# SJTU-ViSYS-team/Avoid-MPC

Hardware: AMD Instinct MI355X
Metric: MPC steps/sec (50k-pt cloud, N=20, 8 obstacle constraints) (higher is better)
Workload: dtype f64; 1 GPU; BASELINE configs[1] batched as configs[2]: 256 scenes/GPU x (50000-pt obstacle cloud + 5000-pt edge cloud, N=20, K=8), fresh frame + zero warm start every step, every in-flight step on its own frames; scenes_per_gpu=256, points=50000, horizon=20, K=8, mpc_max_iter=3, ipm_max_iter=100, streams_in_flight=10, steps_per_launch=4, scenes_per_launch=1024, distinct_frames_bytes=6758400000, hw_queues=4, tie_order=lowest index, parallelism=single GPU, no process group, rccl=no process group (single GPU, plain run): RCCL not used

## Files before the change

avoid_mpc_amd/capi.py:

```python
import ctypes as C
import os

HERE = os.path.dirname(os.path.abspath(__file__))
LIB_PATH = os.path.join(HERE, "libavoid_mpc_amd.so")

AMK_OK, AMK_ERR_INVALID_ARG, AMK_ERR_HIP, AMK_ERR_NO_DEVICE, AMK_ERR_UNSUPPORTED, AMK_ERR_TIMEOUT = 0, 1, 2, 3, 4, 5
AMK_TIES_LOWEST_INDEX, AMK_TIES_NANOFLANN, AMK_TIES_AUTO = 0, 1, 2
AMK_EXACT_OFF, AMK_EXACT_IN_USE, AMK_EXACT_GAVE_UP, AMK_EXACT_TOO_DEEP = -1, 0, 1, 2
AMK_EXACT_NOT_NEEDED = 3
AMK_MAX_K = 64
AMK_MAX_QUERIES = 64
AMK_MAX_HORIZON = 32
AMK_MAX_OUTER_ITER = 8
AMK_MPC_DEFAULT_MAX_ITER = 100

PLUGIN_FUNCTIONS = ["nlp", "nlp_f", "nlp_g", "nlp_grad_f", "nlp_jac_g", "nlp_hess_l", "nlp_grad"]
PLUGIN_HELPERS = ["alloc_mem", "init_mem", "free_mem", "checkout", "release", "incref", "decref", "n_in", "n_out",
                  "default_in", "name_in", "name_out", "sparsity_in", "sparsity_out", "work"]
PLUGIN_SYMBOLS = [f for f in PLUGIN_FUNCTIONS] + [f + "_" + h for f in PLUGIN_FUNCTIONS for h in PLUGIN_HELPERS] + \
                 ["amk_plugin_configure", "amk_plugin_dims"]

SYMBOLS = [
    "amk_version", "amk_status_string", "amk_last_hip_error", "amk_device_count",
    "amk_kd_create", "amk_kd_destroy", "amk_kd_build", "amk_kd_build_pair", "amk_kd_sizes", "amk_kd_search",
# ... 244 lines not shown
        "amk_shard_rccl_info": (i, [C.c_char_p, i, C.POINTER(i), C.POINTER(i)]),
        "amk_shard_wait": (i, [vp, vp, d]),
        "amk_depth_out_size": (i, [i, i, d, C.POINTER(i), C.POINTER(i)]),
        "amk_depth_to_cloud": (i, [vp, i, i, i, C.c_longlong, i, C.POINTER(DepthParams), vp, vp, i, C.c_longlong, vp, vp]),
        "amk_depth_to_cloud_host": (i, [vp, i, i, i, C.c_longlong, i, C.POINTER(DepthParams), vp, vp, i, C.c_longlong, vp]),
        "amk_depth_to_edge_cloud": (i, [vp, i, i, i, C.c_longlong, i, C.POINTER(DepthParams), vp, vp, i, C.c_longlong, vp, vp]),
        "amk_depth_to_edge_cloud_host": (i, [vp, i, i, i, C.c_longlong, i, C.POINTER(DepthParams), vp, vp, i, C.c_longlong, vp]),
        "amk_depth_clouds_work_bytes": (i, [i, i, d, i, C.POINTER(C.c_longlong)]),
        "amk_depth_to_clouds": (i, [vp, i, i, i, C.c_longlong, i, C.POINTER(DepthParams), vp, vp, vp, C.c_longlong, vp, vp, C.c_longlong, vp,
                                    i, vp, C.c_longlong, vp]),
        "amk_depth_to_clouds_host": (i, [vp, i, i, i, C.c_longlong, i, C.POINTER(DepthParams), vp, vp, vp, C.c_longlong, vp, vp, C.c_longlong,
                                         vp, i]),
        "amk_sim_render_depth": (i, [vp, vp, i, i, d, d, C.POINTER(DepthParams), i, i, vp, vp, i, vp]),
        "amk_sim_render_depth_host": (i, [vp, vp, i, i, d, d, C.POINTER(DepthParams), i, i, vp, vp, i]),
        "amk_sim_vehicle_step": (i, [vp, vp, vp, vp, i, d, vp]),
        "amk_sim_vehicle_step_host": (i, [vp, vp, vp, vp, i, d]),
        "amk_sim_render_world": (i, [vp, vp, i, vp, vp, i, i, d, d, C.POINTER(DepthParams), i, i, vp, vp, i, vp]),
        "amk_sim_render_world_host": (i, [vp, vp, i, vp, vp, i, i, d, d, C.POINTER(DepthParams), i, i, vp, vp, i]),
        "amk_sim_vehicle_step_att": (i, [vp, vp, vp, vp, i, d, i, d, vp]),
        "amk_sim_vehicle_step_att_host": (i, [vp, vp, vp, vp, i, d, i, d]),
    }
    sig["amk__kd_set_mode"] = (i, [vp, i])
    sig["amk__sweep_set_target"] = (None, [i])
    sig["amk__sweep_set_order"] = (None, [i])
    sig["amk__frames_force_wide"] = (None, [i])
    sig["amk__mpc_ref_states"] = (i, [vp, vp, ll])
    sig["amk__kfmap_slots_host"] = (i, [vp, vp, vp, vp, vp, vp])
    sig["amk__mpc_dynamics"] = (i, [vp, vp, d, vp, vp, vp, vp])
    sig["amk__depth_set_band_rows"] = (i, [i])
    sig["amk__sim_render_t"] = (i, [vp, vp, i, i, d, d, C.POINTER(DepthParams), i, i, vp, vp, vp])
    sig["amk__sim_chunk"] = (i, [])
    sig["amk__sim_render_world_t"] = (i, [vp, vp, i, vp, vp, i, i, d, d, C.POINTER(DepthParams), i, i, vp, vp, vp])
    sig["amk__sim_world_chunk"] = (i, [])
    for name, (res, args) in sig.items():
        fn = getattr(lib, name, None)
        if fn is None:
            continue
        fn.restype = res
        fn.argtypes = args
    _lib = lib
    return lib


def missing_symbols():
    lib = load()
    return [s for s in SYMBOLS if not hasattr(lib, s)]


def check(status, what=""):
    if status != AMK_OK:
        lib = load()
        msg = lib.amk_status_string(status).decode()
        raise AmkError(f"{what}: {msg} (status {status}, hipError {lib.amk_last_hip_error()})")


def hip_memcpy_dtoh(host_array, dev_ptr):
    import torch
    hip = C.CDLL(os.path.join(os.path.dirname(torch.__file__), "lib", "libamdhip64.so"))
    hip.hipMemcpy.restype = C.c_int
    hip.hipMemcpy.argtypes = [C.c_void_p, C.c_void_p, C.c_size_t, C.c_int]
    return hip.hipMemcpy(host_array.ctypes.data_as(C.c_void_p), C.c_void_p(dev_ptr), host_array.nbytes, 2)


def check_hip(err, what=""):
    if err != 0:
        raise AmkError(f"{what}: hipError {err}")
# ... 30 lines not shown
```

avoid_mpc_amd/csrc/kd_grid.h:

```cpp
#pragma once
#include <cfloat>
#include <type_traits>
#include "kd_device.h"

namespace amk {

#ifndef AMK_GRID_MAX_CELLS
#define AMK_GRID_MAX_CELLS 1024
#endif
constexpr int kGridMaxCells = AMK_GRID_MAX_CELLS;
#ifndef AMK_GRID_PPC
#define AMK_GRID_PPC 64
#endif
constexpr int kGridPointsPerCell = AMK_GRID_PPC;
#ifndef AMK_BUILD_THREADS
#define AMK_BUILD_THREADS 512
#endif
constexpr int kGridBuildThreads = AMK_BUILD_THREADS;
constexpr int kCompactThreads = kGridBuildThreads;
#ifndef AMK_GRID_UNROLL
#define AMK_GRID_UNROLL 16
#endif
constexpr int kGridUnroll = AMK_GRID_UNROLL;
constexpr int kGridParamDoubles = 8;

__device__ __forceinline__ bool finite3(float x, float y, float z) {
    return fabsf(x) <= FLT_MAX && fabsf(y) <= FLT_MAX && fabsf(z) <= FLT_MAX;
}
__device__ __forceinline__ bool boxable3(float x, float y, float z) {
    return fabsf(x) <= 3.0e38f && fabsf(y) <= 3.0e38f && fabsf(z) <= 3.0e38f;
}

__device__ __forceinline__ int cell_of(double p, double bbmin, double inv_h, int g) {
    double c = floor((p - bbmin) * inv_h);
    c = c < 0.0 ? 0.0 : c;
    const double gm = (double)(g - 1);
    c = c > gm ? gm : c;
    return (int)c;
}

__device__ __forceinline__ void grid_geometry(const float *bbox6, int npoints, double *geo, double *gp) {
    double lo[3], hi[3], ext[3], emax = 0.0;
    for (int a = 0; a < 3; ++a) {
        float m0 = bbox6[a], m1 = bbox6[3 + a];
        if (!(m1 >= m0)) { m0 = 0.f; m1 = 0.f; }
        lo[a] = m0; hi[a] = m1;
        ext[a] = (double)m1 - (double)m0;
        emax = fmax(emax, ext[a]);
    }
    const double efloor = fmax(emax * 1e-6, 1e-30);
    double vol = 1.0;
    for (int a = 0; a < 3; ++a) vol *= fmax(ext[a], efloor);
// ... 78 lines not shown
                const int c = hist[i0 + j];
                hist[i0 + j] = run;
                cs[i0 + j] = run;
                run += c;
            }
        if (tid == 0) cs[ncell + 1] = n;
    }
    for (int tt = 1; tt < ntiles; ++tt)
        for (int i = tid; i <= ncell + 1; i += kGridBuildThreads) cs[(size_t)tt * (kGridMaxCells + 2) + i] = n;
    __syncthreads();
    for (int i0 = tid; i0 < n; i0 += kGridUnroll * kGridBuildThreads) {
        float x[kGridUnroll], y[kGridUnroll], z[kGridUnroll];
#pragma unroll
        for (int j = 0; j < kGridUnroll; ++j) {
            const int i = i0 + j * kGridBuildThreads;
            const int ii = i < n ? i : i0;
            x[j] = xs[ii]; y[j] = ys[ii]; z[j] = zs[ii];
        }
#pragma unroll
        for (int j = 0; j < kGridUnroll; ++j) {
            const int i = i0 + j * kGridBuildThreads;
            if (i < n) {
                const int pos = atomicAdd(&hist[cell_id(x[j], y[j], z[j])], 1);
                gpt4[pos] = make_float4(x[j], y[j], z[j], __int_as_float(i));
            }
        }
    }
}

#ifndef AMK_TILE_P
#define AMK_TILE_P 8
#endif
constexpr int kTileP = AMK_TILE_P;
constexpr int kTilePoints = kGridBuildThreads * kTileP;
#ifndef AMK_STAGE_RECORDS
#define AMK_STAGE_RECORDS 4096
#endif
constexpr int kStageRecords = AMK_STAGE_RECORDS;
__host__ __device__ constexpr int grid_tiles(int max_points) { return max_points <= 0 ? 1 : (max_points + kTilePoints - 1) / kTilePoints; }

__device__ __forceinline__ void grid_build_tiles_scene(int s, const float *__restrict__ src, int stride, int cap, int nvis,
                                                       const float *__restrict__ bbox, float4 *__restrict__ GP,
                                                       int *__restrict__ cell_start, int ntiles, double *__restrict__ gparams,
                                                       int *__restrict__ size_out, float *__restrict__ pmax_out,
                                                       float *__restrict__ soa_x = nullptr, float *__restrict__ soa_y = nullptr,
                                                       float *__restrict__ soa_z = nullptr) {
    const int tid = threadIdx.x, lane = tid & 63, w = tid >> 6;
    constexpr int NW = kGridBuildThreads / 64;
    float4 *gpt4 = GP + (size_t)s * cap;
    int *cs_all = cell_start + (size_t)s * ntiles * (kGridMaxCells + 2);
    double *gp = gparams + (size_t)s * kGridParamDoubles;
    __shared__ int hist[kGridMaxCells + 2];
    __shared__ int wsum[NW];
    __shared__ int wcnt[kTileP * NW + 1];
    __shared__ float4 stage[kStageRecords];
    __shared__ float wmax[NW];
    __shared__ double geo[kGridParamDoubles];
    if (tid == 0) grid_geometry(bbox + 6 * s, nvis, geo, gp);
    __syncthreads();
    const double b0 = geo[0], b1 = geo[1], b2 = geo[2], inv_h = geo[4];
    const int g0 = (int)geo[5], g1 = (int)geo[6], g2 = (int)geo[7];
    const int ncell = g0 * g1 * g2;
    float amax = 0.f;
    int kept_before = 0;
    int t = 0;
    for (int i0 = 0; i0 < nvis; i0 += kTilePoints, ++t) {
        int *cs = cs_all + (size_t)t * (kGridMaxCells + 2);
        float x[kTileP], y[kTileP], z[kTileP];
#pragma unroll
        for (int j = 0; j < kTileP; ++j) {
            const int i = i0 + j * kGridBuildThreads + tid;
            const float *q = src + (size_t)(i < nvis ? i : i0) * stride;
            x[j] = q[0]; y[j] = q[1]; z[j] = q[2];
        }
        for (int i = tid; i <= ncell + 1; i += kGridBuildThreads) hist[i] = 0;
        unsigned cell2[kTileP / 2];
        unsigned keepbits = 0;
#pragma unroll
        for (int j = 0; j < kTileP; ++j) {
            const int i = i0 + j * kGridBuildThreads + tid;
            const bool keep = i < nvis && !(x[j] != x[j]);
            const unsigned long long m = __ballot(keep);
            if (lane == 0) wcnt[j * NW + w] = __popcll(m);
            keepbits |= keep ? 1u << j : 0u;
            if (keep) amax = fmaxf(amax, fmaxf(fabsf(x[j]), fmaxf(fabsf(y[j]), fabsf(z[j]))));
            unsigned c = finite3(x[j], y[j], z[j])
                             ? (cell_of(z[j], b2, inv_h, g2) * g1 + cell_of(y[j], b1, inv_h, g1)) * g0 + cell_of(x[j], b0, inv_h, g0)
                             : ncell;
            asm volatile("" : "+v"(c));
            cell2[j / 2] = (j & 1) ? (cell2[j / 2] | c << 16) : c;
        }
        __syncthreads();
#pragma unroll
        for (int j = 0; j < kTileP; ++j)
            if (keepbits >> j & 1) atomicAdd(&hist[cell2[j / 2] >> (16 * (j & 1)) & 0xffffu], 1);
        if (w == 0) {
            constexpr int PER = (kTileP * NW + 63) / 64;
            int loc[PER], sum = 0;
#pragma unroll
            for (int e = 0; e < PER; ++e) {
                const int k = lane * PER + e;
                loc[e] = k < kTileP * NW ? wcnt[k] : 0;
                sum += loc[e];
            }
            int incl = sum;
#pragma unroll
            for (int off = 1; off < 64; off <<= 1) {
                const int v = __shfl_up(incl, off);
                if (lane >= off) incl += v;
            }
            int run = incl - sum;
#pragma unroll
            for (int e = 0; e < PER; ++e) {
                const int k = lane * PER + e;
                if (k < kTileP * NW) wcnt[k] = run;
                run += loc[e];
            }
            if (lane == 63) wcnt[kTileP * NW] = incl;
        }
        __syncthreads();
        const int kept_tile = wcnt[kTileP * NW];
        {
            const int per = (ncell + 1 + kGridBuildThreads - 1) / kGridBuildThreads;
            const int c0 = tid * per;
            int loc = 0;
            for (int j = 0; j < per; ++j)
                if (c0 + j <= ncell) loc += hist[c0 + j];
            int incl = loc;
#pragma unroll
            for (int off = 1; off < 64; off <<= 1) {
                const int v = __shfl_up(incl, off);
                if (lane >= off) incl += v;
            }
            if (lane == 63) wsum[w] = incl;
            __syncthreads();
            int wbase = 0;
            for (int j = 0; j < w; ++j) wbase += wsum[j];
            int run = kept_before + wbase + incl - loc;
            for (int j = 0; j < per; ++j)
                if (c0 + j <= ncell) {
                    const int c = hist[c0 + j];
                    hist[c0 + j] = run;
                    cs[c0 + j] = run;
                    run += c;
                }
            if (tid == 0) cs[ncell + 1] = kept_before + kept_tile;
        }
        __syncthreads();
#pragma unroll
        for (int j = 0; j < kTileP; ++j) {
            unsigned r = 0;
            if (keepbits >> j & 1) r = (unsigned)(atomicAdd(&hist[cell2[j / 2] >> (16 * (j & 1)) & 0xffffu], 1) - kept_before);
            cell2[j / 2] = (j & 1) ? ((cell2[j / 2] & 0xffffu) | r << 16) : ((cell2[j / 2] & 0xffff0000u) | r);
        }
        for (int h0 = 0; h0 < kept_tile; h0 += kStageRecords) {
#pragma unroll
            for (int j = 0; j < kTileP; ++j) {
                const bool keep = keepbits >> j & 1;
                const unsigned long long m = __ballot(keep);
                const int r = (int)(cell2[j / 2] >> (16 * (j & 1)) & 0xffffu) - h0;
                if (keep && r >= 0 && r < kStageRecords) {
                    const int idx = kept_before + wcnt[j * NW + w] + __popcll(m & ((1ull << lane) - 1ull));
                    stage[r] = make_float4(x[j], y[j], z[j], __int_as_float(idx));
                    if (soa_x) { soa_x[idx] = x[j]; soa_y[idx] = y[j]; soa_z[idx] = z[j]; }
                }
            }
            __syncthreads();
            const int nrec = min(kStageRecords, kept_tile - h0);
            for (int i = tid; i < nrec; i += kGridBuildThreads) gpt4[kept_before + h0 + i] = stage[i];
            __syncthreads();
        }
        kept_before += kept_tile;
        __syncthreads();
    }
    if (soa_x) {
        const float qnan = __builtin_nanf("");
        for (int i = kept_before + tid; i < cap; i += kGridBuildThreads) { soa_x[i] = qnan; soa_y[i] = qnan; soa_z[i] = qnan; }
    }
    for (int tt = t; tt < ntiles; ++tt) {
        int *cs = cs_all + (size_t)tt * (kGridMaxCells + 2);
        for (int i = tid; i <= ncell + 1; i += kGridBuildThreads) cs[i] = kept_before;
    }
#pragma unroll
    for (int off = 32; off > 0; off >>= 1) amax = fmaxf(amax, __shfl_xor(amax, off));
    if (lane == 0) wmax[w] = amax;
    __syncthreads();
    if (tid == 0) {
        float mx = 0.f;
        for (int j = 0; j < NW; ++j) mx = fmaxf(mx, wmax[j]);
        *size_out = kept_before;
        *pmax_out = mx;
    }
}

struct GridScene {
    const float4 *pt;
    const int *cs;
    const double *gp;
    int nt;
};

__device__ __forceinline__ int grid_trash_count(const GridScene &gs) {
    const int ncell = (int)gs.gp[5] * (int)gs.gp[6] * (int)gs.gp[7];
    int n = 0;
    for (int t = 0; t < gs.nt; ++t) {
        const int *cst = gs.cs + (size_t)t * (kGridMaxCells + 2);
        n += cst[ncell + 1] - cst[ncell];
    }
    return n;
}

struct GridPtrs {
    const float4 *pt;
    const int *cs;
// ... 969 lines not shown
```

avoid_mpc_amd/csrc/kd_index.hip:

```cpp
#include "kd_exact.h"

#include <cstring>

namespace amk {
thread_local int g_last_hip_error = 0;

struct Timing {
    int mode = 0;
    struct Rec { int kclass; hipEvent_t a, b; };
    std::vector<Rec> recs;
    std::vector<hipEvent_t> pool;
    hipEvent_t get() {
        if (!pool.empty()) { hipEvent_t e = pool.back(); pool.pop_back(); return e; }
        hipEvent_t e;
        (void)hipEventCreate(&e);
        return e;
    }
};
Timing &timing() { static Timing t; return t; }

TimedLaunch::TimedLaunch(int kclass, hipStream_t s) : slot(-1), stream(s) {
    Timing &t = timing();
    if (t.mode == 0 || (t.mode == 1 && kclass != KC_SOLVE && kclass != KC_GRID)) return;
    Timing::Rec r{kclass, t.get(), t.get()};
// ... 9 lines not shown
extern "C" void amk__timing_enable(int mode) { amk::timing().mode = mode; }
extern "C" int amk__timing_collect(double *ms, int *counts) {
    amk::Timing &t = amk::timing();
    for (int i = 0; i < amk::KC_COUNT; ++i) { ms[i] = 0.0; counts[i] = 0; }
    for (auto &r : t.recs) {
        float f = 0.f;
        if (hipEventSynchronize(r.b) != hipSuccess || hipEventElapsedTime(&f, r.a, r.b) != hipSuccess) return AMK_ERR_HIP;
        ms[r.kclass] += f;
        counts[r.kclass] += 1;
        t.pool.push_back(r.a);
        t.pool.push_back(r.b);
    }
    t.recs.clear();
    return AMK_OK;
}

extern "C" int amk__timing_timeline(int max_recs, int *kclass, double *start_ms, double *end_ms) {
    amk::Timing &t = amk::timing();
    int n = 0;
    for (auto &r : t.recs) {
        float fa = 0.f, fb = 0.f;
        if (hipEventSynchronize(r.b) != hipSuccess || hipEventElapsedTime(&fa, t.recs[0].a, r.a) != hipSuccess ||
            hipEventElapsedTime(&fb, t.recs[0].a, r.b) != hipSuccess)
            return AMK_ERR_HIP;
        if (n < max_recs) { kclass[n] = r.kclass; start_ms[n] = fa; end_ms[n] = fb; ++n; }
    }
    for (auto &r : t.recs) { t.pool.push_back(r.a); t.pool.push_back(r.b); }
    t.recs.clear();
    return n;
}

using amk::kWave;

using amk::kCompactThreads;

__device__ __forceinline__ void sample_bbox_scene(int s, const float *__restrict__ src, int point_stride, int n,
                                                  float *__restrict__ bbox_out) {
    const int tid = threadIdx.x, lane = tid & 63, w = tid >> 6;
    constexpr int NW = kCompactThreads / kWave;
    __shared__ float wave_bb[6][NW];
#ifndef AMK_BBOX_STEP
#define AMK_BBOX_STEP 16
#endif
    const int step = n >= 16384 ? AMK_BBOX_STEP : 1;
    float bmn[3] = {3.0e38f, 3.0e38f, 3.0e38f}, bmx[3] = {-3.0e38f, -3.0e38f, -3.0e38f};
    for (int t = tid;; t += kCompactThreads) {
        const long long i = (long long)(t >> 6) * (64 * step) + (t & 63);
        if (i >= n) break;
        const float *p = src + (size_t)i * point_stride;
        const float px = p[0], py = p[1], pz = p[2];
        if (amk::boxable3(px, py, pz)) {
            bmn[0] = fminf(bmn[0], px); bmx[0] = fmaxf(bmx[0], px);
            bmn[1] = fminf(bmn[1], py); bmx[1] = fmaxf(bmx[1], py);
            bmn[2] = fminf(bmn[2], pz); bmx[2] = fmaxf(bmx[2], pz);
        }
    }
#pragma unroll
    for (int off = 32; off > 0; off >>= 1)
#pragma unroll
        for (int a = 0; a < 3; ++a) {
            bmn[a] = fminf(bmn[a], __shfl_xor(bmn[a], off));
            bmx[a] = fmaxf(bmx[a], __shfl_xor(bmx[a], off));
        }
    if (lane == 0)
#pragma unroll
        for (int a = 0; a < 3; ++a) { wave_bb[a][w] = bmn[a]; wave_bb[3 + a][w] = bmx[a]; }
    __syncthreads();
    if (tid < 6) {
        float v = wave_bb[tid][0];
        for (int j = 1; j < NW; ++j) v = tid < 3 ? fminf(v, wave_bb[tid][j]) : fmaxf(v, wave_bb[tid][j]);
        bbox_out[6 * s + tid] = v;
    }
    __threadfence_block();
    __syncthreads();
}

struct BuildArgs {
    const float *xyz;
    int point_stride;
    long long scene_stride;
    const int *counts;
    int max_points, cap;
    int *size_out;
    float *pmax_out, *bbox_out;
    float4 *GP;
    int *cell_start;
    int ntiles;
    double *gparams;
    const int *keep_if_zero;
    float *soa_x, *soa_y, *soa_z;
    const int *out_scene;
};
constexpr int kBuildMaxEntries = 2 * AMK_PIPELINE_MAX_GANG;
struct BuildArgs2 { BuildArgs t[kBuildMaxEntries]; };
__global__ __launch_bounds__(kCompactThreads, 4) void kd_build_kernel(const BuildArgs2 args) {
    const BuildArgs &a = args.t[blockIdx.y];
    const int s_in = blockIdx.x;
    if (a.keep_if_zero && a.keep_if_zero[s_in] == 0) return;
    const int s = a.out_scene ? a.out_scene[s_in] : s_in;
    if (s < 0) return;
    const float *src = a.xyz + (long long)s_in * a.scene_stride;
    int n = a.counts ? a.counts[s_in] : a.max_points;
    n = n < 0 ? 0 : (n > a.max_points ? a.max_points : n);
    sample_bbox_scene(s, src, a.point_stride, n, a.bbox_out);
    const size_t so = (size_t)s * a.cap;
    amk::grid_build_tiles_scene(s, src, a.point_stride, a.cap, n, a.bbox_out, a.GP, a.cell_start, a.ntiles, a.gparams,
                                a.size_out + s, a.pmax_out + s, a.soa_x ? a.soa_x + so : nullptr, a.soa_y ? a.soa_y + so : nullptr,
                                a.soa_z ? a.soa_z + so : nullptr);
}
static BuildArgs build_args(amk_kd *kd, const float *d_xyz, int point_stride, long long scene_stride, const int *d_counts,
                            size_t so = 0) {
    return BuildArgs{d_xyz, point_stride, scene_stride, d_counts, kd->max_points, kd->cap,
                     kd->size.p + so, kd->pmax.p + so, kd->bbox.p + so * 6, kd->gpt.p + so * kd->cap,
                     kd->cell_start.p + so * kd->ntiles * (amk::kGridMaxCells + 2), kd->ntiles,
                     kd->gparams.p + so * amk::kGridParamDoubles, nullptr, nullptr, nullptr, nullptr, nullptr};
}
static bool build_writes_soa(amk_kd *kd, BuildArgs &a, size_t so = 0) {
    if (kd->tie_order != AMK_TIES_NANOFLANN || kd->cap <= 0) return false;
    if (!kd->x.p || !kd->y.p || !kd->z.p) {
        const size_t tot = (size_t)kd->n_scenes * kd->cap;
        if ((!kd->x.p && kd->x.alloc(tot) != hipSuccess) || (!kd->y.p && kd->y.alloc(tot) != hipSuccess) ||
            (!kd->z.p && kd->z.alloc(tot) != hipSuccess))
            return false;
    }
    a.soa_x = kd->x.p + so * kd->cap; a.soa_y = kd->y.p + so * kd->cap; a.soa_z = kd->z.p + so * kd->cap;
    return true;
}

namespace amk {
int kd_build_mapped_gang(amk_kd *obs_pool, amk_kd *edge_pool, int n_frames, int frame_scenes, const float *const *d_xyz,
                         const int *const *d_counts, const float *const *d_edge_xyz, const int *const *d_edge_counts, int point_stride,
                         const int *d_out_scene, hipStream_t stream) {
    if (!obs_pool || !edge_pool || n_frames < 1 || n_frames > AMK_PIPELINE_MAX_GANG || frame_scenes < 1 || !d_out_scene || point_stride < 3)
        return AMK_ERR_INVALID_ARG;
    const int st = pool_planes(obs_pool);
    if (st != AMK_OK) return st;
    BuildArgs2 args{};
    for (int f = 0; f < n_frames; ++f) {
        if (!d_xyz[f] || !d_edge_xyz[f]) return AMK_ERR_INVALID_ARG;
        BuildArgs a = build_args(obs_pool, d_xyz[f], point_stride, (long long)obs_pool->max_points * point_stride, d_counts[f]);
        BuildArgs b = build_args(edge_pool, d_edge_xyz[f], point_stride, (long long)edge_pool->max_points * point_stride, d_edge_counts[f]);
        a.out_scene = b.out_scene = d_out_scene + (size_t)f * frame_scenes;
        a.soa_x = obs_pool->x.p; a.soa_y = obs_pool->y.p; a.soa_z = obs_pool->z.p;
        if (edge_pool->pool_exact) { b.soa_x = edge_pool->x.p; b.soa_y = edge_pool->y.p; b.soa_z = edge_pool->z.p; }
        args.t[2 * f] = a; args.t[2 * f + 1] = b;
    }
    {
        amk::TimedLaunch tg(amk::KC_GRID, stream);
        hipLaunchKernelGGL(kd_build_kernel, dim3(frame_scenes, 2 * n_frames), dim3(kCompactThreads), 0, stream, args);
    }
    AMK_HIP(hipGetLastError());
    for (amk_kd *kd : {obs_pool, edge_pool}) { kd->soa_valid = 0; kd->ex_valid = 0; kd->async_pending = 1; }
    return AMK_OK;
}
int kd_build_mapped(amk_kd *obs_pool, amk_kd *edge_pool, int n_in, const float *d_xyz, const int *d_counts,
                    const float *d_edge_xyz, const int *d_edge_counts, int point_stride, const int *d_out_scene,
                    hipStream_t stream) {
    return kd_build_mapped_gang(obs_pool, edge_pool, 1, n_in, &d_xyz, &d_counts, &d_edge_xyz, &d_edge_counts, point_stride,
                                d_out_scene, stream);
}
}

__global__ __launch_bounds__(256) void kd_records_to_soa_kernel(const float4 *__restrict__ GP, const int *__restrict__ sizes,
                                                                float *__restrict__ X, float *__restrict__ Y,
                                                                float *__restrict__ Z, int cap) {
    const int s = blockIdx.y, i = blockIdx.x * 256 + threadIdx.x;
    if (i >= cap) return;
    const size_t base = (size_t)s * cap;
    if (i < sizes[s]) {
        const float4 r = GP[base + i];
        const int idx = __float_as_int(r.w);
        X[base + idx] = r.x; Y[base + idx] = r.y; Z[base + idx] = r.z;
    } else {
        const float qnan = __builtin_nanf("");
        X[base + i] = qnan; Y[base + i] = qnan; Z[base + i] = qnan;
    }
}

int ensure_soa(amk_kd *kd, hipStream_t stream) {
    if (kd->soa_valid) return AMK_OK;
    if (const int st = amk::pool_planes(kd); st != AMK_OK) return st;
    if (kd->cap > 0)
// ... 76 lines not shown

__global__ __launch_bounds__(256) void kd_tie_flags_kernel(amk::GridPtrs gpt, const int *__restrict__ sizes, int n_scenes,
    const double *__restrict__ queries, int query_stride, int n_queries, int k, int *__restrict__ out_flags) {
    __shared__ amk::GridWaveLds wl[4];
    const amk::WaveSlot m = amk::wave_slot(n_queries);
    if (m.s >= n_scenes || m.unit >= n_queries) return;
    const size_t row = (size_t)m.s * n_queries + m.unit;
    const double *qp = queries + row * query_stride;
    double ld;
    int li, lpos;
    amk::grid_knn(gpt.scene(m.s), qp[0], qp[1], qp[2], k + 1, ld, li, lpos, &wl[m.w]);
    const bool any = amk::wave_tie(ld, li, m.lane, amk::adaptor_count(sizes[m.s], k));
    if (m.lane == 0) out_flags[row] = any;
}

extern "C" int amk_kd_points_host(amk_kd *kd, float *h_xyz, int *h_sizes) {
    if (!kd || !h_xyz || !h_sizes) return AMK_ERR_INVALID_ARG;
    AMK_HIP(hipDeviceSynchronize());
    if (const int st = ensure_soa(kd, nullptr); st != AMK_OK) return st;
    int st = amk::read_back({{h_sizes, kd->size.p, sizeof(int) * kd->n_scenes}});
    for (int s = 0; s < kd->n_scenes && st == AMK_OK; ++s) {
        const size_t at = (size_t)s * kd->cap;
        st = amk::planes_to_xyz(kd->x.p + at, kd->y.p + at, kd->z.p + at, h_sizes[s], h_xyz + (size_t)s * kd->max_points * 3);
    }
    return st;
}

extern "C" int amk__kd_set_mode(amk_kd *kd, int mode) {
    if (!kd) return AMK_ERR_INVALID_ARG;
    kd->mode = mode;
    return AMK_OK;
}

extern "C" {

int amk_version(void) { return 100; }

const char *amk_status_string(int status) {
    switch (status) {
        case AMK_OK: return "ok";
        case AMK_ERR_INVALID_ARG: return "invalid argument";
        case AMK_ERR_HIP: return "HIP runtime error";
        case AMK_ERR_NO_DEVICE: return "no HIP device (this library has no CPU fallback)";
        case AMK_ERR_UNSUPPORTED: return "unsupported size";
        case AMK_ERR_TIMEOUT: return "timed out waiting for a collective (amk_shard_wait)";
        default: return "unknown status";
    }
}

int amk_last_hip_error(void) { return amk::g_last_hip_error; }

int amk_device_count(void) {
    int n = 0;
    if (hipGetDeviceCount(&n) != hipSuccess) return 0;
    return n;
}

int amk_kd_create(int n_scenes, int max_points, amk_kd **out) {
    if (!out || n_scenes <= 0 || max_points < 0) return AMK_ERR_INVALID_ARG;
    *out = nullptr;
    if (amk_device_count() <= 0) return AMK_ERR_NO_DEVICE;
    amk_kd *kd = new amk_kd();
    kd->n_scenes = n_scenes;
    kd->max_points = max_points;
    kd->cap = amk::round_up(max_points, 256) + 1024;
    const size_t tot = (size_t)n_scenes * kd->cap;
// ... 1 lines not shown
    if ((e = kd->size.alloc(n_scenes)) != hipSuccess ||
        (e = kd->pmax.alloc(n_scenes)) != hipSuccess || (e = hipMemset(kd->pmax.p, 0, sizeof(float) * n_scenes)) != hipSuccess) {
        delete kd;
        return amk::hip_fail(e);
    }
    if ((e = hipMemset(kd->size.p, 0, sizeof(int) * n_scenes)) != hipSuccess ||
        (e = kd->gpt.alloc(tot)) != hipSuccess || (e = kd->bbox.alloc((size_t)n_scenes * 6)) != hipSuccess ||
        (e = kd->cell_start.alloc((size_t)n_scenes * (kd->ntiles = amk::grid_tiles(max_points)) * (amk::kGridMaxCells + 2))) != hipSuccess ||
        (e = kd->gparams.alloc((size_t)n_scenes * amk::kGridParamDoubles)) != hipSuccess ||
        (e = hipMemset(kd->cell_start.p, 0, sizeof(int) * (size_t)n_scenes * kd->ntiles * (amk::kGridMaxCells + 2))) != hipSuccess ||
        (e = hipMemset(kd->gparams.p, 0, sizeof(double) * (size_t)n_scenes * amk::kGridParamDoubles)) != hipSuccess) {
        delete kd;
        return amk::hip_fail(e);
    }
    *out = kd;
    return AMK_OK;
}

int amk_kd_destroy(amk_kd *kd) {
    if (!kd) return AMK_ERR_INVALID_ARG;
    delete kd;
    return AMK_OK;
}

int amk_kd_build(amk_kd *kd, const float *d_xyz, int point_stride, long long scene_stride,
                 const int *d_counts, void *stream) {
    if (!kd || (!d_xyz && kd->max_points > 0) || point_stride < 3 || scene_stride < 0) return AMK_ERR_INVALID_ARG;
    {
        amk::TimedLaunch tg(amk::KC_GRID, (hipStream_t)stream);
        BuildArgs a = build_args(kd, d_xyz, point_stride, scene_stride, d_counts);
        const bool soa = build_writes_soa(kd, a);
        BuildArgs2 args{};
        args.t[0] = a;
        hipLaunchKernelGGL(kd_build_kernel, dim3(kd->n_scenes, 1), dim3(kCompactThreads), 0, (hipStream_t)stream, args);
        kd->soa_valid = soa ? 1 : 0;
        kd->ex_valid = 0;
        kd->async_pending = 1;
    }
    AMK_HIP(hipGetLastError());
    return exact_after_index_build(kd, (hipStream_t)stream);
}

int amk_kd_build_pair(amk_kd *obstacle, const float *d_xyz, const int *d_counts, amk_kd *edge, const float *d_edge_xyz,
                      const int *d_edge_counts, int point_stride, void *stream) {
    if (!obstacle || !edge || (!d_xyz && obstacle->max_points > 0) || (!d_edge_xyz && edge->max_points > 0)) return AMK_ERR_INVALID_ARG;
    return amk::kd_build_gang(obstacle, edge, 1, obstacle->n_scenes, &d_xyz, &d_counts, &d_edge_xyz, &d_edge_counts, point_stride,
                              (hipStream_t)stream);
}

}
namespace amk {
int kd_build_gang(amk_kd *obstacle, amk_kd *edge, int n_frames, int frame_scenes, const float *const *d_xyz,
                  const int *const *d_counts, const float *const *d_edge_xyz, const int *const *d_edge_counts, int point_stride,
                  hipStream_t stream, const int *const *d_keep_if_zero) {
    if (!obstacle || !edge || n_frames < 1 || n_frames > AMK_PIPELINE_MAX_GANG || point_stride < 3 ||
        obstacle->n_scenes < n_frames * frame_scenes || edge->n_scenes != obstacle->n_scenes)
        return AMK_ERR_INVALID_ARG;
    {
        amk::TimedLaunch tg(amk::KC_GRID, stream);
        BuildArgs2 args{};
        for (int f = 0; f < n_frames; ++f) {
            const size_t so = (size_t)f * frame_scenes;
            args.t[2 * f] = build_args(obstacle, d_xyz[f], point_stride, (long long)obstacle->max_points * point_stride, d_counts[f], so);
            args.t[2 * f + 1] = build_args(edge, d_edge_xyz[f], point_stride, (long long)edge->max_points * point_stride, d_edge_counts[f], so);
            if (d_keep_if_zero) args.t[2 * f].keep_if_zero = args.t[2 * f + 1].keep_if_zero = d_keep_if_zero[f];
        }
        bool soa_o = !d_keep_if_zero, soa_e = !d_keep_if_zero;
        for (int f = 0; f < n_frames; ++f) {
            soa_o = soa_o && build_writes_soa(obstacle, args.t[2 * f], (size_t)f * frame_scenes);
            soa_e = soa_e && build_writes_soa(edge, args.t[2 * f + 1], (size_t)f * frame_scenes);
        }
        if (!soa_o) for (int f = 0; f < n_frames; ++f) args.t[2 * f].soa_x = args.t[2 * f].soa_y = args.t[2 * f].soa_z = nullptr;
        if (!soa_e) for (int f = 0; f < n_frames; ++f) args.t[2 * f + 1].soa_x = args.t[2 * f + 1].soa_y = args.t[2 * f + 1].soa_z = nullptr;
        hipLaunchKernelGGL(kd_build_kernel, dim3(frame_scenes, 2 * n_frames), dim3(kCompactThreads), 0, stream, args);
        obstacle->soa_valid = soa_o ? 1 : 0; edge->soa_valid = soa_e ? 1 : 0;
        for (amk_kd *kd : {obstacle, edge}) {
            kd->ex_valid = 0;
            kd->async_pending = 1;
        }
    }
    AMK_HIP(hipGetLastError());
    for (amk_kd *kd : {obstacle, edge})
        if (const int st = exact_after_index_build(kd, stream); st != AMK_OK) return st;
    return AMK_OK;
}
}
extern "C" {
int amk_kd_sizes(amk_kd *kd, int *h_sizes, void *stream) {
    if (!kd || !h_sizes) return AMK_ERR_INVALID_ARG;
    AMK_HIP(hipMemcpyAsync(h_sizes, kd->size.p, sizeof(int) * kd->n_scenes, hipMemcpyDeviceToHost, (hipStream_t)stream));
    AMK_HIP(hipStreamSynchronize((hipStream_t)stream));
    return AMK_OK;
}

int amk_kd_search(amk_kd *kd, const double *d_queries, int n_queries, int k, int *d_indices, double *d_sqdist,
                  float *d_pts, int *d_counts, void *stream) {
    if (!kd || !d_queries || n_queries <= 0 || k <= 0) return AMK_ERR_INVALID_ARG;
    if (k > AMK_MAX_K || n_queries > AMK_MAX_QUERIES) return AMK_ERR_UNSUPPORTED;
    if (kd->mode == 0 && kd->tie_order == AMK_TIES_AUTO && k + 1 > AMK_MAX_K) return AMK_ERR_UNSUPPORTED;
    if (kd->auto_on()) {
        hipLaunchKernelGGL(kd_grid_search_auto_kernel, dim3((unsigned)amk::search_blocks(kd->n_scenes, n_queries)), dim3(256), 0, (hipStream_t)stream, grid_ptrs(kd), kd->size.p,
                           kd->n_scenes, d_queries, n_queries, k, d_indices, d_sqdist, d_pts, d_counts, kd->au_rowflag.p, kd->au_need());
        AMK_HIP(hipGetLastError());
        if (const int st = amk::kd_auto_build(kd, nullptr, (hipStream_t)stream); st != AMK_OK) return st;
        return exact_search(kd, d_queries, n_queries, k, d_indices, d_sqdist, d_pts, d_counts, (hipStream_t)stream);
    }
    if (kd->mode == 0) {
// ... 87 lines not shown
```

avoid_mpc_amd/csrc/mpc_solve.hip:

```cpp
#include "mpc_handle.h"

#include <cmath>
#include <algorithm>
#include <cstring>
#include <utility>
#include <vector>

using namespace amk;

extern "C" int amk__mpc_dynamics(const double *tau, const double *drag, double dt, double *A, double *B, double *c, double *dtau) {
    if (!tau || !drag || !A || !B || !c) return AMK_ERR_INVALID_ARG;
    mpc_dynamics(tau, drag, dt, A, B, c, dtau);
    return AMK_OK;
}

namespace {

void refresh_dynamics(amk_mpc *m) {
    amk__mpc_dynamics(m->h_prm + PRM_TAU, m->drag, m->dt, m->h_prm + PRM_A, m->h_prm + PRM_B, m->h_prm + PRM_C, nullptr);
}

int build_plan(amk_mpc *m, std::vector<double> &coef, std::vector<int> &meta) {
    const double *A = m->h_prm + PRM_A, *B = m->h_prm + PRM_B;
    const LdsMap L(m->N);
// ... 239 lines not shown
    if (max_passes > 0) {
        if (!d_done || !d_step_flags) return AMK_ERR_INVALID_ARG;
        if (!m->resume_rec.p) AMK_HIP(m->resume_rec.alloc((size_t)m->S * (8 * m->N + 8)));
        sched = SolveSched{budget > 0 ? budget : 0, max_passes, m->resume_rec.p, const_cast<int *>(d_done)};
    }
    TimedLaunch tl(KC_SOLVE, stream);
    with_horizon(m->N, [&](auto nt) {
        constexpr int NT = decltype(nt)::value;
        auto launch = [&](auto kernel, size_t lds) {
            hipLaunchKernelGGL(kernel, dim3(m->launch_scenes()), dim3(64), lds, stream, m->N, m->K, m->nref, m->nx, m->prm.p, m->opt,
                               d_ref_states, m->w0.p, d_u, d_x0array, d_info, g_trace, d_done, d_ref_path, d_step_flags,
                               m->plan_coef.p, m->plan_meta.p, m->ybuf.p, m->gains.p, sched);
        };
        if (m->precision == 32) launch(mpc_solve_kernel_f32<NT>, m->lds_bytes / 2);
        else launch(mpc_solve_kernel<NT>, m->lds_bytes);
    });
    AMK_HIP(hipGetLastError());
    return AMK_OK;
}
}

extern "C" int amk__plan_dump(amk_mpc *m, int *h_meta, int n_ints) {
    std::vector<double> coef;
    std::vector<int> meta;
    int st = build_plan(m, coef, meta);
    if (st != AMK_OK) return st;
    const LdsMap L(m->N);
    const int hdr[8] = {L.P, L.p, L.lam, L.M, L.Hm, L.G, L.q, L.total};
    for (int i = 0; i < 8 && i < n_ints; ++i) h_meta[i] = hdr[i];
    for (int i = 0; i + 8 < n_ints && i < (int)meta.size(); ++i) h_meta[8 + i] = meta[i];
    return (int)meta.size() + 8;
}

extern "C" int amk__solve_occupancy(amk_mpc *m) {
    int nb = -1;
    const void *f = solve_kernel_f64(m->N);
    hipFuncAttributes fa;
    if (hipFuncGetAttributes(&fa, f) == hipSuccess)
        printf("solve kernel N=%d: numRegs %d, sharedSizeBytes %zu, localSizeBytes %zu, maxDynamicShared %d, lds request %zu\n", m->N,
               fa.numRegs, fa.sharedSizeBytes, fa.localSizeBytes, fa.maxDynamicSharedSizeBytes, m->lds_bytes);
    if (hipOccupancyMaxActiveBlocksPerMultiprocessor(&nb, f, 64, m->lds_bytes) != hipSuccess) return -2;
    return nb;
}

extern "C" {

int amk_mpc_create(double T, double dt, int nearest_point_num, int n_scenes, amk_mpc **out) {
    if (!out || !(T > 0) || !(dt > 0) || nearest_point_num < 0 || n_scenes <= 0) return AMK_ERR_INVALID_ARG;
    *out = nullptr;
    const int N = (int)(T / dt);
    if (N < 2 || N > AMK_MAX_HORIZON || nearest_point_num > AMK_MAX_K) return AMK_ERR_UNSUPPORTED;
    if (amk_device_count() <= 0) return AMK_ERR_NO_DEVICE;
    amk_mpc *m = new amk_mpc();
    m->T = T; m->dt = dt; m->N = N; m->K = nearest_point_num; m->S = n_scenes;
    m->nx = m->dims().nx();
    m->nref = SceneRecord{N, m->K}.len();
    std::memset(m->h_prm, 0, sizeof m->h_prm);
    const double wdef[25] = {100, 100, 100, 300, 1, 1, 1, 0., 0., 0., 0.0, 10, 10, 30, 0, 1, 1, 0., 0., 0., 1., 1., 1., 1., 1.};
    std::memcpy(m->h_prm + PRM_W, wdef, sizeof wdef);
    const double tdef[4] = {0.01, 0.01, 0.01, 0};
    std::memcpy(m->h_prm + PRM_TAU, tdef, sizeof tdef);
    for (int i = 0; i < 4; ++i) m->h_prm[PRM_GAIN + i] = 1.0;
    const double lb[4] = {-10., -10., 1., -10.}, ub[4] = {10., 10., 20., 10.};
    std::memcpy(m->h_prm + PRM_LB, lb, sizeof lb);
    std::memcpy(m->h_prm + PRM_UB, ub, sizeof ub);
    refresh_dynamics(m);
    m->opt.tol = 1e-4; m->opt.max_iter = AMK_MPC_DEFAULT_MAX_ITER; m->opt.max_ls = 12; m->opt.mu_init = 0.1;
    m->opt.bound_push = 1e-3; m->opt.bound_frac = 1e-3; m->opt.kappa_mu = 0.2; m->opt.kappa_eps = 100.0;
    m->opt.mu_min_fac = 1e-2; m->opt.maj = 1.0; m->opt.tau_min = 0.99;
    m->opt.eta_phi = 1e-8; m->opt.s_max = 100.0; m->opt.kappa_sigma = 1e10;
    m->lds_bytes = sizeof(double) * (size_t)LdsMap(N).total;
    if (m->lds_bytes < (size_t)AMK_SOLVE_LDS_MIN) m->lds_bytes = AMK_SOLVE_LDS_MIN;
    hipError_t e;
    if ((e = m->prm.alloc(PRM_LEN)) != hipSuccess ||
        (e = m->plan_coef.alloc((size_t)PLAN_ITEMS * (PLAN_TERMS + 1) + 64 * 2)) != hipSuccess ||
        (e = m->plan_meta.alloc((size_t)PLAN_ITEMS * (PLAN_TERMS + 4) + 64 * LANE_META_INTS)) != hipSuccess || (e = m->w0.alloc((size_t)n_scenes * m->nx)) != hipSuccess ||
        (e = m->ybuf.alloc((size_t)n_scenes * N * (m->K > 0 ? m->K : 1) * kTermRecord)) != hipSuccess ||
        (e = m->gains.alloc((size_t)n_scenes * N * GAIN_STAGE)) != hipSuccess ||
        (e = hipMemset(m->gains.p, 0, sizeof(double) * (size_t)n_scenes * N * GAIN_STAGE)) != hipSuccess ||
        (e = hipMemset(m->w0.p, 0, sizeof(double) * (size_t)n_scenes * m->nx)) != hipSuccess ||
        (e = hipFuncSetAttribute(solve_kernel_f64(N), hipFuncAttributeMaxDynamicSharedMemorySize, (int)m->lds_bytes)) != hipSuccess) {
        delete m;
        return amk::hip_fail(e);
    }
    int st = upload_params(m);
    if (st != AMK_OK) {
        delete m;
        return st;
    }
    *out = m;
    return AMK_OK;
}

int amk_mpc_destroy(amk_mpc *m) {
    if (!m) return AMK_ERR_INVALID_ARG;
    delete m;
    return AMK_OK;
}

int amk_mpc_horizon(const amk_mpc *m) { return m ? m->N : -1; }
int amk_mpc_nx(const amk_mpc *m) { return m ? m->nx : -1; }
int amk_mpc_ref_len(const amk_mpc *m) { return m ? m->nref : -1; }

int amk_mpc_setup_weights(amk_mpc *m, const double *w) {
    if (!m || !w) return AMK_ERR_INVALID_ARG;
// ... 91 lines not shown
```

Before: 513,000 MPC steps/s.

## Shrink index-build blocks and LDS staging, alias histogram into staging buffer

The kd/grid build kernel now runs with its own thread count (256 instead of 512), which also halves the tile size. The LDS staging window drops from 4096 to 512 float4 records, and the cell histogram now shares that window instead of having its own array. Together these cut LDS per block so more build blocks can be resident per CU. The cost is more staging rounds per tile and an extra barrier to protect the aliased histogram. Small query hooks for build shape and solve LDS size are also added.

```diff
diff --git a/avoid_mpc_amd/capi.py b/avoid_mpc_amd/capi.py
--- a/avoid_mpc_amd/capi.py
+++ b/avoid_mpc_amd/capi.py
@@ -300,6 +300,8 @@
     sig["amk__sim_chunk"] = (i, [])
     sig["amk__sim_render_world_t"] = (i, [vp, vp, i, vp, vp, i, i, d, d, C.POINTER(DepthParams), i, i, vp, vp, vp])
     sig["amk__sim_world_chunk"] = (i, [])
+    sig["amk__kd_build_shape"] = (i, [C.POINTER(C.c_int), C.POINTER(C.c_int), C.POINTER(C.c_int)])
+    sig["amk__solve_lds_bytes"] = (i, [i])
     for name, (res, args) in sig.items():
         fn = getattr(lib, name, None)
         if fn is None:
diff --git a/avoid_mpc_amd/csrc/kd_grid.h b/avoid_mpc_amd/csrc/kd_grid.h
--- a/avoid_mpc_amd/csrc/kd_grid.h
+++ b/avoid_mpc_amd/csrc/kd_grid.h
@@ -18,6 +18,10 @@
 #endif
 constexpr int kGridBuildThreads = AMK_BUILD_THREADS;
 constexpr int kCompactThreads = kGridBuildThreads;
+#ifndef AMK_INDEX_BUILD_THREADS
+#define AMK_INDEX_BUILD_THREADS 256
+#endif
+constexpr int kIndexBuildThreads = AMK_INDEX_BUILD_THREADS;
 #ifndef AMK_GRID_UNROLL
 #define AMK_GRID_UNROLL 16
 #endif
@@ -162,11 +166,13 @@
 #define AMK_TILE_P 8
 #endif
 constexpr int kTileP = AMK_TILE_P;
-constexpr int kTilePoints = kGridBuildThreads * kTileP;
+constexpr int kTilePoints = kIndexBuildThreads * kTileP;
+static_assert(4096 % kTilePoints == 0, "tile edges at every multiple of 4096 points");
 #ifndef AMK_STAGE_RECORDS
-#define AMK_STAGE_RECORDS 4096
+#define AMK_STAGE_RECORDS 512
 #endif
 constexpr int kStageRecords = AMK_STAGE_RECORDS;
+static_assert(kStageRecords % 64 == 0 && kStageRecords > 0, "whole-wavefront stores");
 __host__ __device__ constexpr int grid_tiles(int max_points) { return max_points <= 0 ? 1 : (max_points + kTilePoints - 1) / kTilePoints; }
 
 __device__ __forceinline__ void grid_build_tiles_scene(int s, const float *__restrict__ src, int stride, int cap, int nvis,
@@ -176,14 +182,15 @@
                                                        float *__restrict__ soa_x = nullptr, float *__restrict__ soa_y = nullptr,
                                                        float *__restrict__ soa_z = nullptr) {
     const int tid = threadIdx.x, lane = tid & 63, w = tid >> 6;
-    constexpr int NW = kGridBuildThreads / 64;
+    constexpr int NW = kIndexBuildThreads / 64;
     float4 *gpt4 = GP + (size_t)s * cap;
     int *cs_all = cell_start + (size_t)s * ntiles * (kGridMaxCells + 2);
     double *gp = gparams + (size_t)s * kGridParamDoubles;
-    __shared__ int hist[kGridMaxCells + 2];
+    static_assert(sizeof(float4) * kStageRecords >= sizeof(int) * (kGridMaxCells + 2), "the staging window holds the histogram");
+    __shared__ float4 stage[kStageRecords];
+    int *hist = reinterpret_cast<int *>(stage);
     __shared__ int wsum[NW];
     __shared__ int wcnt[kTileP * NW + 1];
-    __shared__ float4 stage[kStageRecords];
     __shared__ float wmax[NW];
     __shared__ double geo[kGridParamDoubles];
     if (tid == 0) grid_geometry(bbox + 6 * s, nvis, geo, gp);
@@ -199,16 +206,16 @@
         float x[kTileP], y[kTileP], z[kTileP];
 #pragma unroll
         for (int j = 0; j < kTileP; ++j) {
-            const int i = i0 + j * kGridBuildThreads + tid;
+            const int i = i0 + j * kIndexBuildThreads + tid;
             const float *q = src + (size_t)(i < nvis ? i : i0) * stride;
             x[j] = q[0]; y[j] = q[1]; z[j] = q[2];
         }
-        for (int i = tid; i <= ncell + 1; i += kGridBuildThreads) hist[i] = 0;
+        for (int i = tid; i <= ncell + 1; i += kIndexBuildThreads) hist[i] = 0;
         unsigned cell2[kTileP / 2];
         unsigned keepbits = 0;
 #pragma unroll
         for (int j = 0; j < kTileP; ++j) {
-            const int i = i0 + j * kGridBuildThreads + tid;
+            const int i = i0 + j * kIndexBuildThreads + tid;
             const bool keep = i < nvis && !(x[j] != x[j]);
             const unsigned long long m = __ballot(keep);
             if (lane == 0) wcnt[j * NW + w] = __popcll(m);
@@ -251,7 +258,7 @@
         __syncthreads();
         const int kept_tile = wcnt[kTileP * NW];
         {
-            const int per = (ncell + 1 + kGridBuildThreads - 1) / kGridBuildThreads;
+            const int per = (ncell + 1 + kIndexBuildThreads - 1) / kIndexBuildThreads;
             const int c0 = tid * per;
             int loc = 0;
             for (int j = 0; j < per; ++j)
@@ -283,13 +290,14 @@
             if (keepbits >> j & 1) r = (unsigned)(atomicAdd(&hist[cell2[j / 2] >> (16 * (j & 1)) & 0xffffu], 1) - kept_before);
             cell2[j / 2] = (j & 1) ? ((cell2[j / 2] & 0xffffu) | r << 16) : ((cell2[j / 2] & 0xffff0000u) | r);
         }
+        __syncthreads();
         for (int h0 = 0; h0 < kept_tile; h0 += kStageRecords) {
 #pragma unroll
             for (int j = 0; j < kTileP; ++j) {
                 const bool keep = keepbits >> j & 1;
                 const unsigned long long m = __ballot(keep);
-                const int r = (int)(cell2[j / 2] >> (16 * (j & 1)) & 0xffffu) - h0;
-                if (keep && r >= 0 && r < kStageRecords) {
+                const unsigned r = (cell2[j / 2] >> (16 * (j & 1)) & 0xffffu) - (unsigned)h0;
+                if (keep && r < (unsigned)kStageRecords) {
                     const int idx = kept_before + wcnt[j * NW + w] + __popcll(m & ((1ull << lane) - 1ull));
                     stage[r] = make_float4(x[j], y[j], z[j], __int_as_float(idx));
                     if (soa_x) { soa_x[idx] = x[j]; soa_y[idx] = y[j]; soa_z[idx] = z[j]; }
@@ -297,19 +305,18 @@
             }
             __syncthreads();
             const int nrec = min(kStageRecords, kept_tile - h0);
-            for (int i = tid; i < nrec; i += kGridBuildThreads) gpt4[kept_before + h0 + i] = stage[i];
+            for (int i = tid; i < nrec; i += kIndexBuildThreads) gpt4[kept_before + h0 + i] = stage[i];
             __syncthreads();
         }
         kept_before += kept_tile;
-        __syncthreads();
     }
     if (soa_x) {
         const float qnan = __builtin_nanf("");
-        for (int i = kept_before + tid; i < cap; i += kGridBuildThreads) { soa_x[i] = qnan; soa_y[i] = qnan; soa_z[i] = qnan; }
+        for (int i = kept_before + tid; i < cap; i += kIndexBuildThreads) { soa_x[i] = qnan; soa_y[i] = qnan; soa_z[i] = qnan; }
     }
     for (int tt = t; tt < ntiles; ++tt) {
         int *cs = cs_all + (size_t)tt * (kGridMaxCells + 2);
-        for (int i = tid; i <= ncell + 1; i += kGridBuildThreads) cs[i] = kept_before;
+        for (int i = tid; i <= ncell + 1; i += kIndexBuildThreads) cs[i] = kept_before;
     }
 #pragma unroll
     for (int off = 32; off > 0; off >>= 1) amax = fmaxf(amax, __shfl_xor(amax, off));
diff --git a/avoid_mpc_amd/csrc/kd_index.hip b/avoid_mpc_amd/csrc/kd_index.hip
--- a/avoid_mpc_amd/csrc/kd_index.hip
+++ b/avoid_mpc_amd/csrc/kd_index.hip
@@ -65,19 +65,19 @@
 
 using amk::kWave;
 
-using amk::kCompactThreads;
+using amk::kIndexBuildThreads;
 
 __device__ __forceinline__ void sample_bbox_scene(int s, const float *__restrict__ src, int point_stride, int n,
                                                   float *__restrict__ bbox_out) {
     const int tid = threadIdx.x, lane = tid & 63, w = tid >> 6;
-    constexpr int NW = kCompactThreads / kWave;
+    constexpr int NW = kIndexBuildThreads / kWave;
     __shared__ float wave_bb[6][NW];
 #ifndef AMK_BBOX_STEP
 #define AMK_BBOX_STEP 16
 #endif
     const int step = n >= 16384 ? AMK_BBOX_STEP : 1;
     float bmn[3] = {3.0e38f, 3.0e38f, 3.0e38f}, bmx[3] = {-3.0e38f, -3.0e38f, -3.0e38f};
-    for (int t = tid;; t += kCompactThreads) {
+    for (int t = tid;; t += kIndexBuildThreads) {
         const long long i = (long long)(t >> 6) * (64 * step) + (t & 63);
         if (i >= n) break;
         const float *p = src + (size_t)i * point_stride;
@@ -126,7 +126,7 @@
 };
 constexpr int kBuildMaxEntries = 2 * AMK_PIPELINE_MAX_GANG;
 struct BuildArgs2 { BuildArgs t[kBuildMaxEntries]; };
-__global__ __launch_bounds__(kCompactThreads, 4) void kd_build_kernel(const BuildArgs2 args) {
+__global__ __launch_bounds__(kIndexBuildThreads, 4) void kd_build_kernel(const BuildArgs2 args) {
     const BuildArgs &a = args.t[blockIdx.y];
     const int s_in = blockIdx.x;
     if (a.keep_if_zero && a.keep_if_zero[s_in] == 0) return;
@@ -180,7 +180,7 @@
     }
     {
         amk::TimedLaunch tg(amk::KC_GRID, stream);
-        hipLaunchKernelGGL(kd_build_kernel, dim3(frame_scenes, 2 * n_frames), dim3(kCompactThreads), 0, stream, args);
+        hipLaunchKernelGGL(kd_build_kernel, dim3(frame_scenes, 2 * n_frames), dim3(kIndexBuildThreads), 0, stream, args);
     }
     AMK_HIP(hipGetLastError());
     for (amk_kd *kd : {obs_pool, edge_pool}) { kd->soa_valid = 0; kd->ex_valid = 0; kd->async_pending = 1; }
@@ -323,6 +323,14 @@
     return AMK_OK;
 }
 
+extern "C" int amk__kd_build_shape(int *threads, int *tile_points, int *stage_records) {
+    if (!threads || !tile_points || !stage_records) return AMK_ERR_INVALID_ARG;
+    *threads = amk::kIndexBuildThreads;
+    *tile_points = amk::kTilePoints;
+    *stage_records = amk::kStageRecords;
+    return AMK_OK;
+}
+
 extern "C" {
 
 int amk_version(void) { return 100; }
@@ -390,7 +398,7 @@
         const bool soa = build_writes_soa(kd, a);
         BuildArgs2 args{};
         args.t[0] = a;
-        hipLaunchKernelGGL(kd_build_kernel, dim3(kd->n_scenes, 1), dim3(kCompactThreads), 0, (hipStream_t)stream, args);
+        hipLaunchKernelGGL(kd_build_kernel, dim3(kd->n_scenes, 1), dim3(kIndexBuildThreads), 0, (hipStream_t)stream, args);
         kd->soa_valid = soa ? 1 : 0;
         kd->ex_valid = 0;
         kd->async_pending = 1;
@@ -430,7 +438,7 @@
         }
         if (!soa_o) for (int f = 0; f < n_frames; ++f) args.t[2 * f].soa_x = args.t[2 * f].soa_y = args.t[2 * f].soa_z = nullptr;
         if (!soa_e) for (int f = 0; f < n_frames; ++f) args.t[2 * f + 1].soa_x = args.t[2 * f + 1].soa_y = args.t[2 * f + 1].soa_z = nullptr;
-        hipLaunchKernelGGL(kd_build_kernel, dim3(frame_scenes, 2 * n_frames), dim3(kCompactThreads), 0, stream, args);
+        hipLaunchKernelGGL(kd_build_kernel, dim3(frame_scenes, 2 * n_frames), dim3(kIndexBuildThreads), 0, stream, args);
         obstacle->soa_valid = soa_o ? 1 : 0; edge->soa_valid = soa_e ? 1 : 0;
         for (amk_kd *kd : {obstacle, edge}) {
             kd->ex_valid = 0;
diff --git a/avoid_mpc_amd/csrc/mpc_solve.hip b/avoid_mpc_amd/csrc/mpc_solve.hip
--- a/avoid_mpc_amd/csrc/mpc_solve.hip
+++ b/avoid_mpc_amd/csrc/mpc_solve.hip
@@ -295,6 +295,12 @@
     return (int)meta.size() + 8;
 }
 
+static size_t solve_lds_bytes(int N) {
+    const size_t b = sizeof(double) * (size_t)LdsMap(N).total;
+    return b < (size_t)AMK_SOLVE_LDS_MIN ? (size_t)AMK_SOLVE_LDS_MIN : b;
+}
+extern "C" int amk__solve_lds_bytes(int N) { return N < 1 || N > AMK_MAX_HORIZON ? -1 : (int)solve_lds_bytes(N); }
+
 extern "C" int amk__solve_occupancy(amk_mpc *m) {
     int nb = -1;
     const void *f = solve_kernel_f64(m->N);
@@ -332,8 +338,7 @@
     m->opt.bound_push = 1e-3; m->opt.bound_frac = 1e-3; m->opt.kappa_mu = 0.2; m->opt.kappa_eps = 100.0;
     m->opt.mu_min_fac = 1e-2; m->opt.maj = 1.0; m->opt.tau_min = 0.99;
     m->opt.eta_phi = 1e-8; m->opt.s_max = 100.0; m->opt.kappa_sigma = 1e10;
-    m->lds_bytes = sizeof(double) * (size_t)LdsMap(N).total;
-    if (m->lds_bytes < (size_t)AMK_SOLVE_LDS_MIN) m->lds_bytes = AMK_SOLVE_LDS_MIN;
+    m->lds_bytes = solve_lds_bytes(N);
     hipError_t e;
     if ((e = m->prm.alloc(PRM_LEN)) != hipSuccess ||
         (e = m->plan_coef.alloc((size_t)PLAN_ITEMS * (PLAN_TERMS + 1) + 64 * 2)) != hipSuccess ||
```

After: 512,600 MPC steps/s (median of 2 runs). Within noise of the previous version (-0.1%).
